# tikv/tikv

Measured on NVIDIA H100. Metric: coprocessor rows/sec (scan+filter+hash-agg) at 1/2/4/8 H100 vs host-CPU ref, higher is better.
Workload: dtype int64

## Files before the change

__graft_entry__.py:

```python
import os
import shutil
import subprocess
import sys

ROOT = os.path.dirname(os.path.abspath(__file__))
CSRC = os.path.join(ROOT, "tikv_b200", "csrc")
OUT_DIR = os.path.join(ROOT, "tikv_b200", "_build")
NVCC = os.environ.get("NVCC", "/usr/local/cuda/bin/nvcc")
NVCC_FLAGS = ["-gencode", "arch=compute_90a,code=sm_90a", "-lineinfo", "-O3", "-std=c++17", "--expt-relaxed-constexpr",
              "-Xcompiler", "-fPIC", "-Xptxas", "-v"]
SOURCES = ["kernels.cu", "encode.cu", "jit.cu", "engine.cu", "sst.cu"]


def _newer(target, deps):
    if not os.path.exists(target):
        return True
    t = os.path.getmtime(target)
    return any(os.path.getmtime(d) > t for d in deps)


def build(verbose=False):
    os.makedirs(OUT_DIR, exist_ok=True)
    headers = [os.path.join(CSRC, f) for f in os.listdir(CSRC) if f.endswith((".h", ".cuh"))] + [os.path.join(ROOT, "include", "b2_copr.h")]
    def compile_one(src):
        s = os.path.join(CSRC, src)
        o = os.path.join(OUT_DIR, src.replace(".cu", ".o"))
        if _newer(o, [s] + headers):
            cmd = [NVCC] + NVCC_FLAGS + ["-c", s, "-o", o]
            r = subprocess.run(cmd, capture_output=True, text=True)
            with open(o + ".log", "w") as f:
                f.write(r.stdout + r.stderr)
            if verbose or r.returncode:
                sys.stderr.write(r.stdout + r.stderr)
            if r.returncode:
                raise RuntimeError(f"nvcc failed for {src}")
        return o

    from concurrent.futures import ThreadPoolExecutor
    with ThreadPoolExecutor(max_workers=len(SOURCES)) as pool:
        objs = list(pool.map(compile_one, SOURCES))
    lib = os.path.join(OUT_DIR, "libb2copr.so")
    if _newer(lib, objs):
        subprocess.check_call([NVCC, "-shared", "-o", lib] + objs + ["-gencode", "arch=compute_90a,code=sm_90a"])
    subprocess.check_call(["make", "-s", "-C", os.path.join(ROOT, "oracle")])
    sys.path.insert(0, ROOT)
    import tikv_b200
    from tikv_b200 import ffi
    ffi.lib()
    _precompile_plans()


def _precompile_plans():
    import ctypes as C
    import threading
    import bench
    from tikv_b200 import ffi, smoke
    L = ffi.lib()
    plans = [bench.build_plan(n) for n in ("c3", "c2", "c4")] + smoke.plans()
    errs = []

    def one(p):
        n = C.c_int32(0)
        if L.b2_plan_precompile(C.byref(p.c), C.byref(n)) != 0:
            errs.append(L.b2_last_error_message().decode())
# ... 21 lines not shown
```

include/b2_copr.h:

```cpp
#ifndef B2_COPR_H_
#define B2_COPR_H_

#ifdef B2_NVRTC
typedef signed char int8_t; typedef unsigned char uint8_t; typedef short int16_t; typedef unsigned short uint16_t;
typedef int int32_t; typedef unsigned int uint32_t; typedef long long int64_t; typedef unsigned long long uint64_t;
#else
#include <stddef.h>
#include <stdint.h>
#endif

#ifdef __cplusplus
extern "C" {
#endif

#define B2_ABI_VERSION 4

enum {
  B2_OK = 0,
  B2_ERR_STORAGE = 1,
  B2_ERR_KEY_IS_LOCKED = 2,
  B2_ERR_WRITE_CONFLICT = 3,
  B2_ERR_EVALUATE = 4,
  B2_ERR_CORRUPTED = 5,
  B2_ERR_DEADLINE = 6,
// ... 250 lines not shown
uint32_t b2_abi_version(void);
const char* b2_build_info(void);

const char* b2_last_error_message(void);

int32_t b2_check_supported(const b2_dag_plan* plan);
int32_t b2_plan_prepare(const b2_dag_plan* plan, int32_t device);
int32_t b2_plan_precompile(const b2_dag_plan* plan, int32_t* n_compiled);
void b2_jit_counters(uint64_t* nvrtc_compiles, uint64_t* disk_cache_hits);

int32_t b2_exec_open(const b2_dag_plan* plan, const b2_key_range* ranges, uint32_t n_ranges,
                     const b2_region_source* src, const b2_exec_config* cfg, b2_exec** out);
int32_t b2_exec_schema(b2_exec* h, int32_t* field_tps, uint32_t* field_flags, uint32_t* n_inout);
int32_t b2_exec_next_batch(b2_exec* h, uint64_t scan_rows, b2_batch* out);
int32_t b2_exec_collect_stats(b2_exec* h, b2_exec_stats* out);
int32_t b2_exec_next_batch_async(b2_exec* h, uint64_t scan_rows);
int32_t b2_exec_poll(b2_exec* h, b2_batch* out);
typedef struct b2_warning {
  int32_t mysql_code;
  int32_t _pad;
  char message[120];
} b2_warning;
int32_t b2_exec_warnings(b2_exec* h, b2_warning* out, uint32_t cap, uint64_t* count_out);
int32_t b2_exec_last_error(b2_exec* h, b2_error_info* out);
enum { B2_ENCODE_TYPE_DEFAULT = 0, B2_ENCODE_TYPE_CHUNK = 1 };
typedef struct b2_encoded_chunk {
  const uint8_t* rows_data;
  uint64_t len;
  uint64_t n_rows;
  int32_t encode_type;
  int32_t location;
} b2_encoded_chunk;
int32_t b2_exec_encode_batch(b2_exec* h, int32_t encode_type, int32_t location, b2_encoded_chunk* out);
int32_t b2_exec_take_scanned_range(b2_exec* h, const uint8_t** lower, uint32_t* lower_len, const uint8_t** upper, uint32_t* upper_len);
int32_t b2_exec_collect_scanned_rows_per_range(b2_exec* h, uint64_t* rows, uint32_t* n_inout);
int32_t b2_exec_can_be_cached(b2_exec* h);
void b2_exec_close(b2_exec* h);

typedef struct b2_agg_partials {
  uint32_t n_groups;
  uint32_t acc_words;
  int32_t location;
  int32_t has_group;
  const uint64_t* keys;
  const uint8_t* key_null;
  const uint64_t* acc;
  uint64_t max_word_mask;
  uint32_t key_words;
  uint32_t _pad;
} b2_agg_partials;
int32_t b2_exec_agg_partials(b2_exec* h, b2_agg_partials* out);
enum { B2_MERGE_ADD = 0, B2_MERGE_MAX = 1, B2_MERGE_OR = 2, B2_MERGE_XOR = 3, B2_MERGE_FIRST_KEY = 4, B2_MERGE_FIRST_VALUE = 5 };
int32_t b2_exec_agg_word_ops(b2_exec* h, uint8_t* ops, uint32_t* n_inout);

int32_t b2_dag_handle(const b2_dag_plan* plan, const b2_key_range* ranges, uint32_t n_ranges,
                      const b2_region_source* src, const b2_exec_config* cfg,
                      b2_batch* out, b2_exec** out_handle);

typedef struct b2_checksum_response {
  uint64_t checksum;
  uint64_t total_kvs;
  uint64_t total_bytes;
} b2_checksum_response;

int32_t b2_checksum_handle(const b2_key_range* ranges, uint32_t n_ranges,
                           const uint8_t* old_prefix, uint32_t old_prefix_len,
                           const uint8_t* new_prefix, uint32_t new_prefix_len,
                           const b2_region_source* src, const b2_exec_config* cfg,
                           b2_checksum_response* out, b2_exec_stats* stats);

int32_t b2_region_pin(int32_t device, uint64_t region_id, uint64_t data_version, const b2_region_source* host_src, b2_region_source* dev_src);
int32_t b2_region_unpin(int32_t device, uint64_t region_id, uint64_t data_version);
void b2_region_cache_stats(int32_t device, uint64_t* bytes_cached, uint64_t* hits, uint64_t* misses);

typedef struct b2_sst_blocks {
  const uint8_t* data;
  const uint64_t* block_offs;
  uint32_t n_blocks;
  uint32_t trailer_len;
  uint32_t key_prefix_len;
  uint32_t key_suffix_len;
} b2_sst_blocks;

typedef struct b2_sst_stats {
  uint64_t n_entries, key_bytes, val_bytes;
  uint64_t n_restart_intervals;
  uint64_t h2d_bytes;
  float decode_ms;
  uint32_t n_lz4_blocks;
} b2_sst_stats;

typedef struct b2_sst b2_sst;
int32_t b2_sst_decode(int32_t device, int32_t location, const b2_sst_blocks* in, b2_sst** h, b2_cf_block* out, b2_sst_stats* stats);
void b2_sst_free(b2_sst* h);
typedef struct b2_sst_encoded {
  const uint8_t* data;
  const uint64_t* block_offs;
  uint64_t data_len;
  uint32_t n_blocks;
  uint32_t _pad;
} b2_sst_encoded;
int32_t b2_sst_encode(int32_t device, const b2_cf_block* flat_device_block, uint32_t entries_per_block, uint32_t restart_interval,
                      uint32_t key_prefix_len, uint8_t key_prefix_byte, uint32_t key_suffix_len, uint32_t trailer_len,
                      b2_sst** h, b2_sst_encoded* out);

int64_t b2_plan_literal(const b2_dag_plan* plan, char* buf, uint64_t cap);
// ... 42 lines not shown
```

tikv_b200/csrc/engine.cu:

```cuda
#include <cuda_runtime.h>
#include <sys/mman.h>
#include <sys/syscall.h>
#include <unistd.h>

#include <algorithm>
#include <cctype>
#include <ctime>
#include <future>
#include <map>
#include <cstdio>
#include <cstring>
#include <memory>
#include <mutex>
#include <string>
#include <vector>

#include <cub/device/device_scan.cuh>

#include "encode.cuh"
#include "jit.h"
#include "kernels.cuh"
#include "plan_literal.h"
#include "plan_compile.h"

// ... 1815 lines not shown
  uint32_t n = (uint32_t)h->cp.output_offsets.size();
  if (field_tps && field_flags)
    for (uint32_t i = 0; i < n && i < *n_inout; ++i) { field_tps[i] = h->cp.schema[h->cp.output_offsets[i]].field_tp; field_flags[i] = h->cp.schema[h->cp.output_offsets[i]].field_flag; }
  *n_inout = n;
  return B2_OK;
}

int32_t b2_exec_next_batch(b2_exec* h, uint64_t scan_rows, b2_batch* out) { return h->next_batch(scan_rows, out); }

int32_t b2_exec_collect_stats(b2_exec* h, b2_exec_stats* out) {
  h->stats.h2d_bytes = h->h2d_bytes; h->stats.d2h_bytes = h->d2h_bytes;
  *out = h->stats;
  return B2_OK;
}
int32_t b2_exec_last_error(b2_exec* h, b2_error_info* out) { *out = h->last_err; return B2_OK; }
int32_t b2_exec_can_be_cached(b2_exec* h) { return (h->check_newer && !h->met_newer_any && !h->saw_lock) ? 1 : 0; }
int32_t b2_exec_take_scanned_range(b2_exec* h, const uint8_t** lower, uint32_t* lower_len, const uint8_t** upper, uint32_t* upper_len) {
  if (!h || !lower || !lower_len || !upper || !upper_len) { g_last_error = "null argument"; return B2_ERR_INVALID_ARG; }
  return h->take_scanned_range(lower, lower_len, upper, upper_len);
}
int32_t b2_exec_collect_scanned_rows_per_range(b2_exec* h, uint64_t* rows, uint32_t* n_inout) {
  if (!h || !n_inout) { g_last_error = "null argument"; return B2_ERR_INVALID_ARG; }
  return h->collect_scanned_rows_per_range(rows, n_inout);
}
int32_t b2_exec_encode_batch(b2_exec* h, int32_t encode_type, int32_t location, b2_encoded_chunk* out) {
  if (!h || !out) { g_last_error = "null argument"; return B2_ERR_INVALID_ARG; }
  return h->encode_batch(encode_type, location, out);
}
void b2_exec_close(b2_exec* h) {
  if (h && h->async_running) h->async_fut.wait();
  delete h;
}

int32_t b2_exec_agg_partials(b2_exec* h, b2_agg_partials* out) {
  if (h->cp.dev.mode != PM_AGG || !h->drained) { g_last_error = "no aggregation state: not an Aggregation pipeline or not drained yet"; return B2_ERR_INVALID_ARG; }
  out->n_groups = h->part_n; out->acc_words = (uint32_t)h->cp.dev.acc_words; out->location = B2_LOC_DEVICE; out->has_group = h->cp.dev.has_group;
  out->keys = (const uint64_t*)h->part_keys; out->key_null = (const uint8_t*)h->part_null; out->acc = (const uint64_t*)h->part_acc;
  out->max_word_mask = 0;
  out->key_words = (uint32_t)std::max(1, h->cp.dev.n_group); out->_pad = 0;
  for (int a = 0; a < h->cp.dev.n_aggs; ++a)
    if (agg_is_extremum(h->cp.dev.aggs[a].kind)) out->max_word_mask |= 1ull << (h->cp.dev.aggs[a].acc_off + 1);
  return B2_OK;
}
int32_t b2_exec_agg_word_ops(b2_exec* h, uint8_t* ops, uint32_t* n_inout) {
  if (!h || !ops || !n_inout) { g_last_error = "null argument"; return B2_ERR_INVALID_ARG; }
  if (h->cp.dev.mode != PM_AGG || !h->drained) { g_last_error = "no aggregation state: not an Aggregation pipeline or not drained yet"; return B2_ERR_INVALID_ARG; }
  const uint32_t n = (uint32_t)h->cp.dev.acc_words;
  if (*n_inout < n) { *n_inout = n; g_last_error = "ops buffer smaller than acc_words"; return B2_ERR_INVALID_ARG; }
  for (uint32_t w = 0; w < n; ++w) ops[w] = (uint8_t)agg_word_op(h->cp.dev, (int)w);
  *n_inout = n;
  return B2_OK;
}

int32_t b2_dag_handle(const b2_dag_plan* plan, const b2_key_range* ranges, uint32_t n_ranges, const b2_region_source* src,
                      const b2_exec_config* cfg, b2_batch* out, b2_exec** out_handle) {
  b2_exec* h = nullptr;
  int rc = b2_exec_open(plan, ranges, n_ranges, src, cfg, &h);
  if (rc) return rc;
  *out_handle = h;
  if (h->paging_size) {
    const uint64_t budget = std::min<uint64_t>(std::max<uint64_t>(h->paging_size * 2, 64), 1ull << 24);
    rc = h->next_batch(budget, out);
    if (rc == B2_OK && out->is_drained == B2_DRAIN_REMAIN) out->is_drained = B2_DRAIN_PAGING;
    return rc;
  }
  return h->next_batch(~0ull, out);
}

int32_t b2_exec_next_batch_async(b2_exec* h, uint64_t scan_rows) {
  if (!h) { g_last_error = "null argument"; return B2_ERR_INVALID_ARG; }
  if (h->async_running) { g_last_error = "a batch is already in flight on this handle"; return B2_ERR_INVALID_ARG; }
  h->async_running = true;
  h->async_fut = std::async(std::launch::async, [h, scan_rows] { return h->next_batch(scan_rows, &h->async_batch); });
  return B2_OK;
}
int32_t b2_exec_poll(b2_exec* h, b2_batch* out) {
  if (!h || !out) { g_last_error = "null argument"; return B2_ERR_INVALID_ARG; }
  if (!h->async_running) { g_last_error = "no batch in flight"; return B2_ERR_INVALID_ARG; }
  if (h->async_fut.wait_for(std::chrono::seconds(0)) != std::future_status::ready) return B2_PENDING;
  const int rc = h->async_fut.get();
  h->async_running = false;
  *out = h->async_batch;
  if (rc) g_last_error = h->last_err.message;
  return rc;
}

int32_t b2_exec_warnings(b2_exec* h, b2_warning* out, uint32_t cap, uint64_t* count_out) {
  if (!h || !count_out) { g_last_error = "null argument"; return B2_ERR_INVALID_ARG; }
  *count_out = h->warnings_total;
  const uint64_t n = std::min<uint64_t>(std::min<uint64_t>(h->warnings_total, cap), 64);
  for (uint64_t i = 0; out && i < n; ++i) {
    out[i].mysql_code = B2_MYSQL_ERR_DIVISION_BY_ZERO; out[i]._pad = 0;
    snprintf(out[i].message, sizeof(out[i].message), "Division by 0");
  }
  return B2_OK;
}

namespace {
struct PinnedRegion {
  std::vector<DevBuf> bufs;
  std::vector<b2_cf_block> write, dflt;
  b2_cf_block lock{};
  std::vector<std::vector<uint8_t>> lock_host;
  std::vector<uint32_t> lock_ko, lock_vo;
  bool has_lock = false;
  uint64_t bytes = 0;
// ... 280 lines not shown
```

tikv_b200/csrc/kernels.cuh:

```cuda
#pragma once
#ifndef B2_NVRTC
#include <cuda_runtime.h>
#endif

#include "b2_device.h"

namespace b2 {

enum { TILE = 256 };

struct Counters {
  unsigned long long err;
  unsigned long long out_rows;
  unsigned long long out_base;
  unsigned long long live_rows;
  unsigned long long processed_keys;
  unsigned long long processed_size;
  unsigned long long entries_scanned;
  unsigned long long default_lookups;
  unsigned long long checksum, total_kvs, total_bytes;
  unsigned int met_newer;
  unsigned int agg_overflow;
  unsigned int n_groups;
  unsigned int bad_prefix;
// ... 87 lines not shown
};

#ifndef B2_NVRTC
cudaError_t launch_scan(const DevPlan& plan, const ScanArgs& a, int grid, size_t smem, cudaStream_t s);
cudaError_t launch_fast(const DevPlan& plan, const ScanArgs& a, int grid, size_t smem, cudaStream_t s);
int fast_max_grid(int mode, size_t smem);
size_t fast_stage_bytes(uint32_t key_cap, uint32_t val_cap);
size_t fast_checksum_bytes();
int scan_max_grid(int mode, size_t smem);
int scan_topn_hbm_max_grid(size_t smem);
cudaError_t launch_scan_topn_hbm(const DevPlan& plan, const ScanArgs& a, int grid, size_t smem, cudaStream_t s);
int scan_num_sms();
size_t scan_stage_bytes(uint32_t key_cap, uint32_t val_cap);
size_t scan_crc_table_bytes();
int scan_kernel_mode(const DevPlan& plan);
size_t scan_out_stage_bytes();
uint32_t scan_stage_entries();
cudaError_t launch_agg_finalize(const DevPlan& plan, const AggTable& t, Counters* ctr, unsigned long long* out_keys, unsigned char* out_key_null,
                                unsigned long long* out_acc, cudaStream_t s);
cudaError_t launch_agg_result(const DevPlan& plan, unsigned int n_groups, const unsigned long long* g_keys, const unsigned char* g_null,
                              const unsigned long long* g_acc, unsigned long long** col_data, unsigned long long** col_bitmap, cudaStream_t s);
cudaError_t launch_topn_merge(const DevPlan& plan, const TopNLists& in, const TopNLists& out, uint32_t fan_in, cudaStream_t s);
cudaError_t launch_topn_gather(const DevPlan& plan, const ScanArgs& a, const TopItem* items, const unsigned int* count, unsigned long long* pay,
                               unsigned char* pay_null, uint32_t stride, cudaStream_t s);
cudaError_t launch_topn_copy(const TopItem* items, const unsigned int* count, uint32_t n_out, uint32_t stride, const unsigned long long* pay0,
                             const unsigned char* null0, const unsigned long long* pay1, const unsigned char* null1, unsigned long long* pay_out,
                             unsigned char* null_out, cudaStream_t s);
cudaError_t launch_topn_merge2(const DevPlan& plan, const TopItem* a, const unsigned int* a_cnt, const TopItem* b, const unsigned int* b_cnt, TopItem* out,
                               unsigned int* out_cnt, uint32_t limit, cudaStream_t s);
cudaError_t launch_pack_nulls(const unsigned char* nulls, uint32_t n_cols, uint32_t stride, uint32_t n, unsigned long long* bitmaps, uint32_t words_per_col, cudaStream_t s);
size_t topn_smem_bytes(uint32_t cap, int n_order);
cudaError_t launch_open_probe(const BlockView* blocks, uint32_t n_wblocks, uint32_t n_blocks, const uint8_t* bounds, const uint32_t* bound_offs, uint32_t n_ranges,
                              uint32_t first_range, uint32_t* out, uint32_t* unit_ok, uint32_t* ends, uint32_t* sample, cudaStream_t s);
cudaError_t launch_gen_sizes(const b2_gen_spec& spec, uint32_t* row_entries, uint32_t* row_val_bytes, cudaStream_t s);
cudaError_t launch_gen_write(const GenArgs& a, cudaStream_t s);
cudaError_t launch_fill_u64(unsigned long long* p, unsigned long long v, size_t n, cudaStream_t s);
enum { MAX_RAW = 16 };
struct RawCol {
  unsigned long long* cells;
  long long* offsets;
  unsigned char* heap;
  unsigned long long* heap_used;
  unsigned long long heap_cap;
};
struct RawArgs {
  RawCol col[MAX_RAW];
  unsigned char var_idx[MAX_RAW], dec_idx[MAX_RAW];
  unsigned int n_var, n_dec;
  const unsigned long long* row_lo; const unsigned long long* row_hi;
  unsigned long long* sums; unsigned long long sums_stride;
  unsigned int* err;
};
cudaError_t launch_raw_materialise(const RawArgs& R, uint64_t max_rows, cudaStream_t s);
cudaError_t launch_reverse_rows(const unsigned long long* in, const unsigned long long* bm_in, uint64_t in_cap, unsigned long long* out, unsigned long long* bm_out,
                                uint64_t out_cap, uint64_t n_rows, uint64_t n_take, uint32_t n_cols, cudaStream_t s);

#endif

}
```

tikv_b200/dist.py:

```python
import torch
import torch.distributed as dist

SIGN = -(1 << 63)


def shard_blocks(n_blocks, world, rank):
    per, rem = divmod(n_blocks, world)
    lo = rank * per + min(rank, rem)
    return list(range(lo, lo + per + (1 if rank < rem else 0)))


def _world():
    return dist.get_world_size() if dist.is_initialized() else 1


def _all_gather_var(t):
    world = _world()
    if world == 1:
        return [t]
    n = torch.tensor([t.shape[0]], dtype=torch.int64, device=t.device)
    sizes = [torch.zeros_like(n) for _ in range(world)]
    dist.all_gather(sizes, n)
    m = int(max(int(s.item()) for s in sizes))
    pad = torch.zeros((m,) + tuple(t.shape[1:]), dtype=t.dtype, device=t.device)
    pad[: t.shape[0]] = t
    out = [torch.zeros_like(pad) for _ in range(world)]
    dist.all_gather(out, pad)
    return [o[: int(s.item())] for o, s in zip(out, sizes)]


F64_ACC_DIGITS = 66


def f64_acc_digits(x):
    import struct
    bits = struct.unpack("<Q", struct.pack("<d", float(x)))[0]
    m, e = bits & ((1 << 52) - 1), (bits >> 52) & 0x7FF
    if e:
        m |= 1 << 52
    else:
        e = 1
    v = (-m if bits >> 63 else m) << (e - 1)
    sign = -1 if v < 0 else 1
    v = abs(v)
    return [sign * ((v >> (32 * i)) & 0xFFFFFFFF) for i in range(F64_ACC_DIGITS)]


def f64_acc_value(words):
    from fractions import Fraction
    total = 0
    for i, w in enumerate(words):
        w = int(w)
        if w >= 1 << 63:
            w -= 1 << 64
        total += w << (32 * i)
    return float(Fraction(total, 1 << 1074))


def merge_agg_partials(keys, key_null, acc, real_words=(), max_words=(), word_ops=None, desc=False):
    from . import ffi
    ops = list(word_ops) if word_ops is not None else []
    max_words = set(max_words) | {w for w, o in enumerate(ops) if o == ffi.MERGE_MAX}
    bit_words = {w: o for w, o in enumerate(ops) if o in (ffi.MERGE_OR, ffi.MERGE_XOR)}
    first_words = [w for w, o in enumerate(ops) if o == ffi.MERGE_FIRST_KEY]
    special = set(real_words) | max_words | set(bit_words) | {w for w, o in enumerate(ops) if o in (ffi.MERGE_FIRST_KEY, ffi.MERGE_FIRST_VALUE)}
    multi = keys.dim() == 2
    kw = keys.shape[1] if multi else 1
    parts = _all_gather_var(torch.cat([keys.view(-1, kw), key_null.to(torch.int64).view(-1, 1), acc], dim=1))
    part_of = torch.cat([torch.full((p.shape[0],), i, dtype=torch.int64, device=p.device) for i, p in enumerate(parts)])
    allp = torch.cat(parts, dim=0)
    if allp.shape[0] == 0:
        return keys[:0], key_null[:0], acc[:0]
    k, nul, a = allp[:, :kw], allp[:, kw], allp[:, kw + 1:]
    if not multi:
        k = torch.where(nul.bool().view(-1, 1), torch.zeros_like(k), k)
    ident = torch.cat([nul.view(-1, 1), k], dim=1)
    uniq, inv = torch.unique(ident, dim=0, return_inverse=True)
    out = torch.zeros((uniq.shape[0], a.shape[1]), dtype=torch.int64, device=a.device)
    ng = uniq.shape[0]
    for w, o in bit_words.items():
        for b0 in range(0, 64, 8):
            shifts = torch.arange(b0, b0 + 8, device=a.device)
            planes = ((a[:, w].view(-1, 1) >> shifts) & 1).to(torch.uint8)
            red = torch.zeros((ng, 8), dtype=torch.uint8, device=a.device)
            if o == ffi.MERGE_OR:
                red.scatter_reduce_(0, inv.view(-1, 1).expand(-1, 8), planes, reduce="amax")
            else:
                red.index_add_(0, inv, planes)
            out[:, w] |= ((red & 1).to(torch.int64) << shifts).sum(dim=1)
    for w in first_words:
        has = a[:, w] != 0
        pref = part_of if desc else len(parts) - 1 - part_of
        pref = torch.where(has, pref, torch.full_like(pref, -1))
        best = torch.full((ng,), -1, dtype=torch.int64, device=a.device).scatter_reduce_(0, inv, pref, reduce="amax")
        cand = has & (pref == best[inv])
        flipped = torch.where(cand, a[:, w] ^ SIGN, torch.full_like(a[:, w], SIGN))
        top = torch.full((ng,), SIGN, dtype=torch.int64, device=a.device).scatter_reduce_(0, inv, flipped, reduce="amax")
        win = cand & (flipped == top[inv])
        out[inv[win], w] = a[win, w]
        out[inv[win], w + 1] = a[win, w + 1]
    int_words = [w for w in range(a.shape[1]) if w not in special]
    if int_words:
        out[:, int_words] = torch.zeros((uniq.shape[0], len(int_words)), dtype=torch.int64, device=a.device).index_add_(0, inv, a[:, int_words])
    for w in real_words:
        s = torch.zeros(uniq.shape[0], dtype=torch.float64, device=a.device).index_add_(0, inv, a[:, w].contiguous().view(torch.float64))
        out[:, w] = s.view(torch.int64)
    for w in max_words:
        flipped = a[:, w] ^ (-(1 << 63))
        m = torch.full((uniq.shape[0],), -(1 << 63), dtype=torch.int64, device=a.device).scatter_reduce_(0, inv, flipped, reduce="amax")
        out[:, w] = m ^ (-(1 << 63))
    if multi:
        return uniq[:, 1:].contiguous(), uniq[:, 0].contiguous(), out
    return uniq[:, 1].contiguous(), uniq[:, 0].bool(), out


def limbs_to_int(lo, hi, unsigned=False):
    lo &= (1 << 64) - 1
    if unsigned:
        hi &= (1 << 64) - 1
    elif hi >= (1 << 63):
        hi -= 1 << 64
    return hi * (1 << 32) + lo


def _order_word(col, null, desc, kind):
# ... 87 lines not shown
```

tikv_b200/ffi.py:

```python
import ctypes as C
import os

_HERE = os.path.dirname(os.path.abspath(__file__))
LIB_PATH = os.path.join(_HERE, "_build", "libb2copr.so")

B2_OK, B2_ERR_STORAGE, B2_ERR_KEY_IS_LOCKED, B2_ERR_WRITE_CONFLICT, B2_ERR_EVALUATE = 0, 1, 2, 3, 4
B2_ERR_CORRUPTED, B2_ERR_DEADLINE, B2_ERR_UNSUPPORTED, B2_ERR_CUDA, B2_ERR_INVALID_ARG = 5, 6, 7, 8, 9
B2_PENDING = 100

TP_TINY, TP_SHORT, TP_LONG, TP_FLOAT, TP_DOUBLE, TP_NULL, TP_TIMESTAMP, TP_LONGLONG, TP_INT24 = 1, 2, 3, 4, 5, 6, 7, 8, 9
TP_DATE, TP_DURATION, TP_DATETIME, TP_YEAR, TP_VARCHAR, TP_BIT = 10, 11, 12, 13, 15, 16
TP_JSON, TP_NEWDECIMAL, TP_ENUM, TP_SET, TP_BLOB, TP_VARSTRING, TP_STRING = 0xF5, 0xF6, 0xF7, 0xF8, 0xFC, 0xFD, 0xFE
FLAG_NOT_NULL, FLAG_UNSIGNED = 1, 32
EXTRA_PHYSICAL_TABLE_ID_COL_ID, EXTRA_COMMIT_TS_COL_ID = -3, -5

LOC_HOST, LOC_DEVICE = 0, 1
ISO_SI, ISO_RC, ISO_RC_CHECK_TS = 0, 1, 2

RPN_CONST_NULL, RPN_CONST_INT, RPN_CONST_UINT, RPN_CONST_REAL, RPN_COLUMN_REF, RPN_FN, RPN_CONST_TIME, RPN_CONST_DURATION, RPN_CONST_BYTES, RPN_CONST_DECIMAL = 0, 1, 2, 3, 4, 5, 6, 7, 8, 9

def _header_enum(prefix):
    import re
    with open(os.path.join(os.path.dirname(_HERE), "include", "b2_copr.h")) as f:
        text = f.read()
# ... 94 lines not shown
    _fields_ = [("status", C.c_int32), ("mysql_code", C.c_int32), ("entry_index", C.c_uint64), ("message", C.c_char * 232)]


class ChecksumResponse(C.Structure):
    _fields_ = [("checksum", C.c_uint64), ("total_kvs", C.c_uint64), ("total_bytes", C.c_uint64)]


class AggPartials(C.Structure):
    _fields_ = [("n_groups", C.c_uint32), ("acc_words", C.c_uint32), ("location", C.c_int32), ("has_group", C.c_int32),
                ("keys", C.c_void_p), ("key_null", C.c_void_p), ("acc", C.c_void_p), ("max_word_mask", C.c_uint64),
                ("key_words", C.c_uint32), ("_pad", C.c_uint32)]


class Warning(C.Structure):
    _fields_ = [("mysql_code", C.c_int32), ("_pad", C.c_int32), ("message", C.c_char * 120)]


class GenSpec(C.Structure):
    _fields_ = [("table_id", C.c_int64), ("first_handle", C.c_uint64), ("n_rows", C.c_uint64), ("n_cols", C.c_uint32),
                ("row_format", C.c_int32), ("seed", C.c_uint64), ("col_lo", C.POINTER(C.c_int64)),
                ("col_range", C.POINTER(C.c_uint64)), ("null_per_million", C.POINTER(C.c_uint32)),
                ("extra_versions_per_million", C.c_uint32), ("delete_per_million", C.c_uint32),
                ("lock_rec_per_million", C.c_uint32), ("commit_ts", C.c_uint64), ("newer_ts", C.c_uint64)]


class GenBlock(C.Structure):
    _fields_ = [("block", CfBlock), ("key_bytes", C.c_uint64), ("val_bytes", C.c_uint64), ("n_user_keys", C.c_uint64)]


class SstBlocks(C.Structure):
    _fields_ = [("data", C.c_void_p), ("block_offs", C.c_void_p), ("n_blocks", C.c_uint32), ("trailer_len", C.c_uint32),
                ("key_prefix_len", C.c_uint32), ("key_suffix_len", C.c_uint32)]


class SstStats(C.Structure):
    _fields_ = [("n_entries", C.c_uint64), ("key_bytes", C.c_uint64), ("val_bytes", C.c_uint64), ("n_restart_intervals", C.c_uint64),
                ("h2d_bytes", C.c_uint64), ("decode_ms", C.c_float), ("n_lz4_blocks", C.c_uint32)]


class SstEncoded(C.Structure):
    _fields_ = [("data", C.c_void_p), ("block_offs", C.c_void_p), ("data_len", C.c_uint64), ("n_blocks", C.c_uint32), ("_pad", C.c_uint32)]


class EncodedChunk(C.Structure):
    _fields_ = [("rows_data", C.c_void_p), ("len", C.c_uint64), ("n_rows", C.c_uint64), ("encode_type", C.c_int32), ("location", C.c_int32)]


ENCODE_TYPE_DEFAULT, ENCODE_TYPE_CHUNK = 0, 1
JIT_AUTO, JIT_SYNC, JIT_OFF = 0, 1, 2

EXPORTED_SYMBOLS = [
    "b2_abi_version", "b2_build_info", "b2_last_error_message", "b2_check_supported", "b2_plan_prepare", "b2_plan_precompile", "b2_jit_counters", "b2_plan_literal", "b2_exec_open", "b2_exec_schema",
    "b2_exec_next_batch", "b2_exec_next_batch_async", "b2_exec_poll", "b2_exec_warnings", "b2_region_pin", "b2_region_unpin", "b2_region_cache_stats", "b2_exec_collect_stats", "b2_exec_last_error", "b2_exec_can_be_cached", "b2_exec_encode_batch", "b2_exec_take_scanned_range", "b2_exec_collect_scanned_rows_per_range", "b2_exec_close",
    "b2_exec_agg_partials", "b2_exec_agg_word_ops", "b2_dag_handle", "b2_checksum_handle", "b2_gen_create", "b2_gen_destroy", "b2_copy_to_host", "b2_copy_to_device",
    "b2_sst_decode", "b2_sst_free", "b2_sst_encode",
    "b2_device_count", "b2_host_alloc_pinned", "b2_host_alloc_pinned_near", "b2_device_numa_node", "b2_host_free_pinned",
]

_lib = None


def lib():
    global _lib
    if _lib is not None:
        return _lib
    if not os.path.exists(LIB_PATH):
        raise RuntimeError(
            f"{LIB_PATH} is missing: the CUDA extension is the product path and there is no CPU fallback. "
            "Run `python -c 'import __graft_entry__ as g; g.build()'` first.")
    L = C.CDLL(LIB_PATH)
    vp, u32, u64, i32 = C.c_void_p, C.c_uint32, C.c_uint64, C.c_int32
    L.b2_abi_version.restype = u32
    L.b2_build_info.restype = C.c_char_p
    L.b2_last_error_message.restype = C.c_char_p
    L.b2_check_supported.argtypes = [C.POINTER(DagPlan)]
    L.b2_check_supported.restype = i32
    L.b2_plan_prepare.argtypes = [C.POINTER(DagPlan), i32]
    L.b2_plan_prepare.restype = i32
    L.b2_plan_precompile.argtypes = [C.POINTER(DagPlan), C.POINTER(i32)]
    L.b2_plan_precompile.restype = i32
    L.b2_jit_counters.argtypes = [C.POINTER(u64), C.POINTER(u64)]
    L.b2_jit_counters.restype = None
    L.b2_exec_open.argtypes = [C.POINTER(DagPlan), C.POINTER(KeyRange), u32, C.POINTER(RegionSource), C.POINTER(ExecConfig), C.POINTER(vp)]
    L.b2_exec_open.restype = i32
    L.b2_exec_schema.argtypes = [vp, C.POINTER(i32), C.POINTER(u32), C.POINTER(u32)]
    L.b2_exec_schema.restype = i32
    L.b2_exec_next_batch.argtypes = [vp, u64, C.POINTER(Batch)]
    L.b2_exec_next_batch.restype = i32
    L.b2_exec_next_batch_async.argtypes = [vp, u64]
    L.b2_exec_next_batch_async.restype = i32
    L.b2_exec_poll.argtypes = [vp, C.POINTER(Batch)]
    L.b2_exec_poll.restype = i32
    L.b2_exec_warnings.argtypes = [vp, C.POINTER(Warning), u32, C.POINTER(u64)]
    L.b2_exec_warnings.restype = i32
    L.b2_region_pin.argtypes = [i32, u64, u64, C.POINTER(RegionSource), C.POINTER(RegionSource)]
    L.b2_region_pin.restype = i32
    L.b2_region_unpin.argtypes = [i32, u64, u64]
    L.b2_region_unpin.restype = i32
    L.b2_region_cache_stats.argtypes = [i32, C.POINTER(u64), C.POINTER(u64), C.POINTER(u64)]
    L.b2_region_cache_stats.restype = None
    L.b2_exec_collect_stats.argtypes = [vp, C.POINTER(ExecStats)]
    L.b2_exec_collect_stats.restype = i32
    L.b2_exec_last_error.argtypes = [vp, C.POINTER(ErrorInfo)]
    L.b2_exec_last_error.restype = i32
    L.b2_exec_encode_batch.argtypes = [vp, i32, i32, C.POINTER(EncodedChunk)]
    L.b2_exec_encode_batch.restype = i32
    L.b2_exec_take_scanned_range.argtypes = [vp, C.POINTER(C.c_void_p), C.POINTER(C.c_uint32), C.POINTER(C.c_void_p), C.POINTER(C.c_uint32)]
    L.b2_exec_take_scanned_range.restype = i32
    L.b2_exec_collect_scanned_rows_per_range.argtypes = [vp, C.POINTER(C.c_uint64), C.POINTER(C.c_uint32)]
    L.b2_exec_collect_scanned_rows_per_range.restype = i32
    L.b2_exec_can_be_cached.argtypes = [vp]
    L.b2_exec_can_be_cached.restype = i32
    L.b2_exec_agg_partials.argtypes = [vp, C.POINTER(AggPartials)]
    L.b2_exec_agg_partials.restype = i32
    L.b2_exec_agg_word_ops.argtypes = [vp, C.POINTER(C.c_uint8), C.POINTER(u32)]
    L.b2_exec_agg_word_ops.restype = i32
    L.b2_exec_close.argtypes = [vp]
    L.b2_exec_close.restype = None
    L.b2_dag_handle.argtypes = [C.POINTER(DagPlan), C.POINTER(KeyRange), u32, C.POINTER(RegionSource), C.POINTER(ExecConfig), C.POINTER(Batch), C.POINTER(vp)]
    L.b2_dag_handle.restype = i32
    L.b2_checksum_handle.argtypes = [C.POINTER(KeyRange), u32, C.c_char_p, u32, C.c_char_p, u32, C.POINTER(RegionSource), C.POINTER(ExecConfig), C.POINTER(ChecksumResponse), C.POINTER(ExecStats)]
    L.b2_checksum_handle.restype = i32
    L.b2_gen_create.argtypes = [i32, C.POINTER(GenSpec), C.POINTER(vp), C.POINTER(GenBlock)]
    L.b2_gen_create.restype = i32
    L.b2_gen_destroy.argtypes = [vp]
    L.b2_gen_destroy.restype = None
    L.b2_sst_decode.argtypes = [i32, i32, C.POINTER(SstBlocks), C.POINTER(vp), C.POINTER(CfBlock), C.POINTER(SstStats)]
    L.b2_sst_decode.restype = i32
    L.b2_sst_free.argtypes = [vp]
    L.b2_sst_free.restype = None
    L.b2_sst_encode.argtypes = [i32, C.POINTER(CfBlock), u32, u32, u32, C.c_uint8, u32, u32, C.POINTER(vp), C.POINTER(SstEncoded)]
    L.b2_sst_encode.restype = i32
    L.b2_copy_to_host.argtypes = [i32, vp, vp, u64]
    L.b2_copy_to_host.restype = i32
    L.b2_copy_to_device.argtypes = [i32, vp, vp, u64]
    L.b2_copy_to_device.restype = i32
    L.b2_device_count.restype = i32
    L.b2_host_alloc_pinned.argtypes = [u64]
    L.b2_host_alloc_pinned.restype = vp
    L.b2_host_alloc_pinned_near.argtypes = [i32, u64]
    L.b2_host_alloc_pinned_near.restype = vp
    L.b2_device_numa_node.argtypes = [i32]
    L.b2_device_numa_node.restype = i32
    L.b2_host_free_pinned.argtypes = [vp]
    L.b2_host_free_pinned.restype = None
    if L.b2_abi_version() != 4:
        raise RuntimeError("libb2copr ABI version mismatch")
    _lib = L
    return L
```

Before: 38.62 billion.

## Merge aggregation partials on device with a native sort-based kernel

Adds a native CUDA path for merging per-device hash-aggregation partials. It radix-sorts rows by their key words (LSD passes), flags group heads, scans to assign group ids, and reduces each group with a warp, including FIRST key/value selection. This replaces the multi-step torch merge whenever the data is on the GPU and no real words are present. It adds several kernel launches, per-call buffer allocation and a host sync in exchange for cutting torch op overhead.

Result: faster. 40.25 billion (median of 6 runs) (+4.2%).

```diff
diff --git a/__graft_entry__.py b/__graft_entry__.py
--- a/__graft_entry__.py
+++ b/__graft_entry__.py
@@ -9,7 +9,7 @@
 NVCC = os.environ.get("NVCC", "/usr/local/cuda/bin/nvcc")
 NVCC_FLAGS = ["-gencode", "arch=compute_90a,code=sm_90a", "-lineinfo", "-O3", "-std=c++17", "--expt-relaxed-constexpr",
               "-Xcompiler", "-fPIC", "-Xptxas", "-v"]
-SOURCES = ["kernels.cu", "encode.cu", "jit.cu", "engine.cu", "sst.cu"]
+SOURCES = ["kernels.cu", "encode.cu", "jit.cu", "engine.cu", "sst.cu", "agg_merge.cu"]
 
 
 def _newer(target, deps):
diff --git a/include/b2_copr.h b/include/b2_copr.h
--- a/include/b2_copr.h
+++ b/include/b2_copr.h
@@ -326,6 +326,10 @@
 int32_t b2_exec_agg_partials(b2_exec* h, b2_agg_partials* out);
 enum { B2_MERGE_ADD = 0, B2_MERGE_MAX = 1, B2_MERGE_OR = 2, B2_MERGE_XOR = 3, B2_MERGE_FIRST_KEY = 4, B2_MERGE_FIRST_VALUE = 5 };
 int32_t b2_exec_agg_word_ops(b2_exec* h, uint8_t* ops, uint32_t* n_inout);
+int32_t b2_agg_merge(int32_t device, uint64_t cuda_stream, uint64_t n_rows, uint32_t key_words, uint32_t acc_words,
+                     const int64_t* keys, uint64_t keys_stride, const uint8_t* key_null, const int64_t* acc, uint64_t acc_stride,
+                     const uint64_t* part_offs, uint32_t n_parts, const uint8_t* ops, int32_t desc,
+                     int64_t* out_keys, uint8_t* out_null, int64_t* out_acc, uint64_t* n_groups);
 
 int32_t b2_dag_handle(const b2_dag_plan* plan, const b2_key_range* ranges, uint32_t n_ranges,
                       const b2_region_source* src, const b2_exec_config* cfg,
diff --git a/tikv_b200/csrc/agg_merge.cu b/tikv_b200/csrc/agg_merge.cu
--- /dev/null
+++ b/tikv_b200/csrc/agg_merge.cu
@@ -0,0 +1,158 @@
+#include <cub/device/device_radix_sort.cuh>
+#include <cub/device/device_scan.cuh>
+
+#include <algorithm>
+
+#include "kernels.cuh"
+
+namespace b2 {
+
+namespace {
+
+__global__ void agg_merge_gather_kernel(AggMergeArgs a, uint32_t word, const unsigned int* perm, unsigned int* perm_out, long long* keys_out) {
+  const uint32_t i = blockIdx.x * blockDim.x + threadIdx.x;
+  if (i >= a.n) return;
+  unsigned int r = i;
+  if (perm) r = perm[i];
+  else perm_out[i] = i;
+  long long v;
+  if (word == a.key_words) v = a.key_null[r];
+  else if (a.key_words == 1 && a.key_null[r]) v = 0;
+  else v = a.keys[(size_t)r * a.keys_stride + word];
+  keys_out[i] = v;
+}
+
+__device__ __forceinline__ bool agg_merge_same_ident(const AggMergeArgs& a, unsigned int r, unsigned int q) {
+  if (a.key_null[r] != a.key_null[q]) return false;
+  if (a.key_words == 1 && a.key_null[r]) return true;
+  for (uint32_t k = 0; k < a.key_words; ++k)
+    if (a.keys[(size_t)r * a.keys_stride + k] != a.keys[(size_t)q * a.keys_stride + k]) return false;
+  return true;
+}
+
+__global__ void agg_merge_heads_kernel(AggMergeArgs a, const unsigned int* perm, unsigned int* flags) {
+  const uint32_t i = blockIdx.x * blockDim.x + threadIdx.x;
+  if (i >= a.n) return;
+  flags[i] = i == 0 || !agg_merge_same_ident(a, perm[i], perm[i - 1]);
+}
+
+__global__ void agg_merge_starts_kernel(const unsigned int* gid, uint32_t n, unsigned int* starts, unsigned int* n_groups) {
+  const uint32_t i = blockIdx.x * blockDim.x + threadIdx.x;
+  if (i >= n) return;
+  const unsigned int g = gid[i];
+  if (g != (i ? gid[i - 1] : 0u)) starts[g - 1] = i;
+  if (i == n - 1) { starts[g] = n; *n_groups = g; }
+}
+
+__device__ __forceinline__ uint32_t agg_merge_part_of(const unsigned long long* part_offs, uint32_t n_parts, unsigned int r) {
+  uint32_t lo = 0, hi = n_parts;
+  while (hi - lo > 1) {
+    const uint32_t mid = (lo + hi) / 2;
+    if (part_offs[mid] <= r) lo = mid; else hi = mid;
+  }
+  return lo;
+}
+
+__device__ __forceinline__ unsigned long long agg_merge_op(unsigned char op, unsigned long long x, unsigned long long y) {
+  if (op == B2_MERGE_ADD) return x + y;
+  if (op == B2_MERGE_MAX) return x > y ? x : y;
+  if (op == B2_MERGE_OR) return x | y;
+  return x ^ y;
+}
+
+__global__ void agg_merge_reduce_kernel(AggMergeArgs a, const unsigned int* perm, const unsigned int* starts, const unsigned int* n_groups) {
+  const uint32_t lane = threadIdx.x & 31, n_warps = gridDim.x * blockDim.x / 32, ng = *n_groups;
+  for (uint32_t g = (blockIdx.x * blockDim.x + threadIdx.x) / 32; g < ng; g += n_warps) {
+    const uint32_t lo = starts[g], hi = starts[g + 1];
+    if (lane == 0) {
+      const long long* first = a.keys + (size_t)perm[lo] * a.keys_stride;
+      const unsigned char mask = a.key_null[perm[lo]];
+      for (uint32_t k = 0; k < a.key_words; ++k) a.out_keys[(size_t)g * a.key_words + k] = (a.key_words == 1 && mask != 0) ? 0 : first[k];
+      a.out_null[g] = mask;
+    }
+    long long* out = a.out_acc + (size_t)g * a.acc_words;
+    for (uint32_t w = 0; w < a.acc_words; ++w) {
+      const long long* col = a.acc + w;
+      const unsigned char op = a.ops[w];
+      if (op == B2_MERGE_FIRST_VALUE) continue;
+      if (op == B2_MERGE_FIRST_KEY) {
+        uint32_t has = 0, pref = 0, pos = 0;
+        unsigned long long key = 0;
+        for (uint32_t j = lo + lane; j < hi; j += 32) {
+          const unsigned long long k = (unsigned long long)col[(size_t)perm[j] * a.acc_stride];
+          if (k == 0) continue;
+          const uint32_t p = agg_merge_part_of(a.part_offs, a.n_parts, perm[j]), pr = a.desc ? p : a.n_parts - 1 - p;
+          if (!has || pr > pref || (pr == pref && k >= key)) { has = 1; pref = pr; key = k; pos = j; }
+        }
+        for (int off = 16; off; off >>= 1) {
+          const uint32_t h2 = __shfl_down_sync(0xffffffffu, has, off), p2 = __shfl_down_sync(0xffffffffu, pref, off), j2 = __shfl_down_sync(0xffffffffu, pos, off);
+          const unsigned long long k2 = __shfl_down_sync(0xffffffffu, key, off);
+          if (h2 && (!has || p2 > pref || (p2 == pref && (k2 > key || (k2 == key && j2 > pos))))) { has = 1; pref = p2; key = k2; pos = j2; }
+        }
+        if (lane == 0) {
+          out[w] = has ? (long long)key : 0;
+          out[w + 1] = has ? col[(size_t)perm[pos] * a.acc_stride + 1] : 0;
+        }
+        continue;
+      }
+      unsigned long long acc = 0;
+      for (uint32_t j = lo + lane; j < hi; j += 32) acc = agg_merge_op(op, acc, (unsigned long long)col[(size_t)perm[j] * a.acc_stride]);
+      for (int off = 16; off; off >>= 1) acc = agg_merge_op(op, acc, __shfl_down_sync(0xffffffffu, acc, off));
+      if (lane == 0) out[w] = (long long)acc;
+    }
+  }
+}
+
+size_t align256(size_t x) { return (x + 255) & ~(size_t)255; }
+
+}
+
+cudaError_t launch_agg_merge(const AggMergeArgs& a, void* tmp, size_t* tmp_bytes, cudaStream_t s) {
+  const uint32_t n = a.n;
+  const size_t keys_b = align256((size_t)n * 8), idx_b = align256((size_t)n * 4), starts_b = align256(((size_t)n + 1) * 4);
+  const size_t fixed = 2 * keys_b + 3 * idx_b + starts_b;
+  cub::DoubleBuffer<long long> kq(nullptr, nullptr);
+  cub::DoubleBuffer<unsigned int> vq(nullptr, nullptr);
+  if (!tmp) {
+    size_t sort_key_b = 0, sort_mask_b = 0, scan_b = 0;
+    cudaError_t e = cub::DeviceRadixSort::SortPairs(nullptr, sort_key_b, kq, vq, (int)n, 0, 64, s);
+    if (e == cudaSuccess) e = cub::DeviceRadixSort::SortPairs(nullptr, sort_mask_b, kq, vq, (int)n, 0, (int)a.key_words, s);
+    if (e == cudaSuccess) e = cub::DeviceScan::InclusiveSum(nullptr, scan_b, (unsigned int*)nullptr, (unsigned int*)nullptr, (int)n, s);
+    *tmp_bytes = fixed + std::max(std::max(sort_key_b, sort_mask_b), scan_b);
+    return e;
+  }
+  if (*tmp_bytes < fixed) return cudaErrorInvalidValue;
+  const size_t cub_b = *tmp_bytes - fixed;
+  cudaError_t e = cudaSuccess;
+  if (n == 0) return cudaMemsetAsync(a.n_groups, 0, 4, s);
+
+  char* p = (char*)tmp;
+  long long* k0 = (long long*)p; p += keys_b;
+  long long* k1 = (long long*)p; p += keys_b;
+  unsigned int* v0 = (unsigned int*)p; p += idx_b;
+  unsigned int* v1 = (unsigned int*)p; p += idx_b;
+  unsigned int* gid = (unsigned int*)p; p += idx_b;
+  unsigned int* starts = (unsigned int*)p; p += starts_b;
+  void* cub_tmp = p;
+  kq = cub::DoubleBuffer<long long>(k0, k1);
+  vq = cub::DoubleBuffer<unsigned int>(v0, v1);
+  const int threads = 256, blocks = (int)((n + threads - 1) / threads);
+  for (uint32_t pass = 0; pass <= a.key_words; ++pass) {
+    const uint32_t word = pass < a.key_words ? a.key_words - 1 - pass : a.key_words;
+    agg_merge_gather_kernel<<<blocks, threads, 0, s>>>(a, word, pass ? vq.Current() : nullptr, vq.Current(), kq.Current());
+    size_t b = cub_b;
+    e = cub::DeviceRadixSort::SortPairs(cub_tmp, b, kq, vq, (int)n, 0, word == a.key_words ? (int)a.key_words : 64, s);
+    if (e != cudaSuccess) return e;
+  }
+  const unsigned int* perm = vq.Current();
+  agg_merge_heads_kernel<<<blocks, threads, 0, s>>>(a, perm, gid);
+  size_t b = cub_b;
+  e = cub::DeviceScan::InclusiveSum(cub_tmp, b, gid, gid, (int)n, s);
+  if (e != cudaSuccess) return e;
+  agg_merge_starts_kernel<<<blocks, threads, 0, s>>>(gid, n, starts, a.n_groups);
+  const int reduce_blocks = (int)(((size_t)n * 32 + threads - 1) / threads < 4096 ? ((size_t)n * 32 + threads - 1) / threads : 4096);
+  agg_merge_reduce_kernel<<<reduce_blocks, threads, 0, s>>>(a, perm, starts, a.n_groups);
+  return cudaGetLastError();
+}
+
+}
diff --git a/tikv_b200/csrc/engine.cu b/tikv_b200/csrc/engine.cu
--- a/tikv_b200/csrc/engine.cu
+++ b/tikv_b200/csrc/engine.cu
@@ -1891,6 +1891,65 @@
   return B2_OK;
 }
 
+int32_t b2_agg_merge(int32_t device, uint64_t cuda_stream, uint64_t n_rows, uint32_t key_words, uint32_t acc_words,
+                     const int64_t* keys, uint64_t keys_stride, const uint8_t* key_null, const int64_t* acc, uint64_t acc_stride,
+                     const uint64_t* part_offs, uint32_t n_parts, const uint8_t* ops, int32_t desc,
+                     int64_t* out_keys, uint8_t* out_null, int64_t* out_acc, uint64_t* n_groups) {
+  if (!part_offs || !n_groups || (acc_words && !ops) ||
+      (n_rows && (!keys || !key_null || !out_keys || !out_null || (acc_words && (!acc || !out_acc))))) {
+    g_last_error = "null argument"; return B2_ERR_INVALID_ARG;
+  }
+  if (key_words < 1 || key_words > 4 || n_rows >= (1ull << 31) || n_parts < 1 || part_offs[0] != 0 || part_offs[n_parts] != n_rows ||
+      keys_stride < key_words || (acc_words && acc_stride < acc_words)) {
+    g_last_error = "b2_agg_merge: 1..4 key words, n_rows < 2^31, n_parts >= 1 offsets from 0 to n_rows, row strides >= the words of a row";
+    return B2_ERR_INVALID_ARG;
+  }
+  for (uint32_t p = 0; p < n_parts; ++p)
+    if (part_offs[p] > part_offs[p + 1]) { g_last_error = "b2_agg_merge: part offsets decrease"; return B2_ERR_INVALID_ARG; }
+  for (uint32_t w = 0; w < acc_words; ++w) {
+    const bool pair_ok = ops[w] == B2_MERGE_FIRST_KEY ? w + 1 < acc_words && ops[w + 1] == B2_MERGE_FIRST_VALUE
+                       : ops[w] == B2_MERGE_FIRST_VALUE ? w > 0 && ops[w - 1] == B2_MERGE_FIRST_KEY : ops[w] <= B2_MERGE_XOR;
+    if (!pair_ok) { g_last_error = "b2_agg_merge: unknown op, or a FIRST key word not followed by its value word"; return B2_ERR_INVALID_ARG; }
+  }
+  *n_groups = 0;
+  if (n_rows == 0) return B2_OK;
+  int prev = -1;
+  cudaGetDevice(&prev);
+  if (cudaSetDevice(device) != cudaSuccess) { g_last_error = "cudaSetDevice failed (the CUDA device path is required; there is no CPU fallback)"; return B2_ERR_CUDA; }
+  struct RestoreDevice { int d; ~RestoreDevice() { if (d >= 0) cudaSetDevice(d); } } restore{prev};
+  const cudaStream_t s = (cudaStream_t)cuda_stream;
+  AggMergeArgs a{};
+  a.keys = (const long long*)keys; a.key_null = key_null; a.acc = (const long long*)acc;
+  a.keys_stride = keys_stride; a.acc_stride = acc_stride; a.n = (uint32_t)n_rows; a.key_words = key_words; a.acc_words = acc_words; a.n_parts = n_parts;
+  a.desc = desc; a.out_keys = (long long*)out_keys; a.out_null = out_null; a.out_acc = (long long*)out_acc;
+  const size_t ops_b = (acc_words + 7) & ~7u, offs_b = ((size_t)n_parts + 1) * 8, up_b = ops_b + offs_b;
+  const size_t count_off = (up_b + 255) & ~(size_t)255, scratch_off = count_off + 256;
+  size_t merge_b = 0;
+  cudaError_t e = launch_agg_merge(a, nullptr, &merge_b, s);
+  HostBuf host;
+  DevBuf dev;
+  if (e == cudaSuccess) e = host.reserve(up_b + 8);
+  if (e == cudaSuccess) e = dev.reserve(scratch_off + merge_b);
+  if (e != cudaSuccess) { g_last_error = std::string("b2_agg_merge buffers: ") + cudaGetErrorString(e); return B2_ERR_CUDA; }
+  uint8_t* hp = (uint8_t*)host.p;
+  if (acc_words) memcpy(hp, ops, acc_words);
+  memcpy(hp + ops_b, part_offs, offs_b);
+  uint8_t* dp = (uint8_t*)dev.p;
+  a.ops = dp; a.part_offs = (const unsigned long long*)(dp + ops_b);
+  a.n_groups = (unsigned int*)(dp + count_off);
+  e = cudaMemcpyAsync(dp, hp, up_b, cudaMemcpyHostToDevice, s);
+  if (e == cudaSuccess) e = launch_agg_merge(a, dp + scratch_off, &merge_b, s);
+  if (e == cudaSuccess) e = cudaMemcpyAsync(hp + up_b, a.n_groups, 4, cudaMemcpyDeviceToHost, s);
+  if (e == cudaSuccess) e = cudaStreamSynchronize(s);
+  if (e != cudaSuccess) {
+    cudaStreamSynchronize(s);
+    g_last_error = std::string("b2_agg_merge: ") + cudaGetErrorString(e);
+    return B2_ERR_CUDA;
+  }
+  *n_groups = *(const unsigned int*)(hp + up_b);
+  return B2_OK;
+}
+
 int32_t b2_dag_handle(const b2_dag_plan* plan, const b2_key_range* ranges, uint32_t n_ranges, const b2_region_source* src,
                       const b2_exec_config* cfg, b2_batch* out, b2_exec** out_handle) {
   b2_exec* h = nullptr;
diff --git a/tikv_b200/csrc/kernels.cuh b/tikv_b200/csrc/kernels.cuh
--- a/tikv_b200/csrc/kernels.cuh
+++ b/tikv_b200/csrc/kernels.cuh
@@ -163,6 +163,21 @@
   unsigned int* err;
 };
 cudaError_t launch_raw_materialise(const RawArgs& R, uint64_t max_rows, cudaStream_t s);
+struct AggMergeArgs {
+  const long long* keys;
+  const unsigned char* key_null;
+  const long long* acc;
+  uint64_t keys_stride, acc_stride;
+  uint32_t n, key_words, acc_words, n_parts;
+  const unsigned char* ops;
+  const unsigned long long* part_offs;
+  int32_t desc;
+  long long* out_keys;
+  unsigned char* out_null;
+  long long* out_acc;
+  unsigned int* n_groups;
+};
+cudaError_t launch_agg_merge(const AggMergeArgs& a, void* tmp, size_t* tmp_bytes, cudaStream_t s);
 cudaError_t launch_reverse_rows(const unsigned long long* in, const unsigned long long* bm_in, uint64_t in_cap, unsigned long long* out, unsigned long long* bm_out,
                                 uint64_t out_cap, uint64_t n_rows, uint64_t n_take, uint32_t n_cols, cudaStream_t s);
 
diff --git a/tikv_b200/dist.py b/tikv_b200/dist.py
--- a/tikv_b200/dist.py
+++ b/tikv_b200/dist.py
@@ -58,19 +58,60 @@
 
 
 def merge_agg_partials(keys, key_null, acc, real_words=(), max_words=(), word_ops=None, desc=False):
+    multi = keys.dim() == 2
+    kw = keys.shape[1] if multi else 1
+    if keys.is_cuda and not real_words:
+        if _world() == 1:
+            return _merge_native(keys.view(-1, kw), key_null, acc, [keys.shape[0]], multi, max_words, word_ops, desc)
+        parts = _all_gather_var(torch.cat([keys.view(-1, kw), key_null.to(torch.int64).view(-1, 1), acc], dim=1))
+        allp = torch.cat(parts, dim=0)
+        return _merge_native(allp[:, :kw], allp[:, kw], allp[:, kw + 1:], [p.shape[0] for p in parts], multi, max_words, word_ops, desc)
+    parts = _all_gather_var(torch.cat([keys.view(-1, kw), key_null.to(torch.int64).view(-1, 1), acc], dim=1))
+    return _merge_gathered_torch(parts, kw, multi, real_words, max_words, word_ops, desc)
+
+
+def _merge_native(keys, key_null, acc, part_sizes, multi, max_words=(), word_ops=None, desc=False):
+    import ctypes as C
+    from . import ffi
+    if keys.stride(1) != 1:
+        keys = keys.contiguous()
+    if acc.shape[1] and acc.stride(1) != 1:
+        acc = acc.contiguous()
+    if key_null.dtype not in (torch.bool, torch.uint8) or not key_null.is_contiguous():
+        key_null = key_null.to(torch.uint8).contiguous()
+    n, kw, aw = keys.shape[0], keys.shape[1], acc.shape[1]
+    ops = list(word_ops) if word_ops is not None else [ffi.MERGE_ADD] * aw
+    for w in max_words:
+        ops[w] = ffi.MERGE_MAX
+    offs = [0]
+    for m in part_sizes:
+        offs.append(offs[-1] + m)
+    out_k = torch.empty((n, kw) if multi else (n,), dtype=torch.int64, device=keys.device)
+    out_n = torch.empty(n, dtype=torch.uint8, device=keys.device)
+    out_a = torch.empty((n, aw), dtype=torch.int64, device=keys.device)
+    ng = C.c_uint64()
+    L = ffi.lib()
+    rc = L.b2_agg_merge(keys.device.index, torch.cuda.current_stream(keys.device).cuda_stream, n, kw, aw,
+                        keys.data_ptr(), keys.stride(0), key_null.data_ptr(), acc.data_ptr(), acc.stride(0) if aw else 0,
+                        (C.c_uint64 * len(offs))(*offs), len(part_sizes), (C.c_uint8 * max(1, aw))(*ops), int(bool(desc)),
+                        out_k.data_ptr(), out_n.data_ptr(), out_a.data_ptr(), C.byref(ng))
+    if rc != 0:
+        raise RuntimeError("b2_agg_merge: " + L.b2_last_error_message().decode())
+    g = ng.value
+    return out_k[:g], (out_n[:g].to(torch.int64) if multi else out_n[:g].view(torch.bool)), out_a[:g]
+
+
+def _merge_gathered_torch(parts, kw, multi, real_words=(), max_words=(), word_ops=None, desc=False):
     from . import ffi
     ops = list(word_ops) if word_ops is not None else []
     max_words = set(max_words) | {w for w, o in enumerate(ops) if o == ffi.MERGE_MAX}
     bit_words = {w: o for w, o in enumerate(ops) if o in (ffi.MERGE_OR, ffi.MERGE_XOR)}
     first_words = [w for w, o in enumerate(ops) if o == ffi.MERGE_FIRST_KEY]
     special = set(real_words) | max_words | set(bit_words) | {w for w, o in enumerate(ops) if o in (ffi.MERGE_FIRST_KEY, ffi.MERGE_FIRST_VALUE)}
-    multi = keys.dim() == 2
-    kw = keys.shape[1] if multi else 1
-    parts = _all_gather_var(torch.cat([keys.view(-1, kw), key_null.to(torch.int64).view(-1, 1), acc], dim=1))
     part_of = torch.cat([torch.full((p.shape[0],), i, dtype=torch.int64, device=p.device) for i, p in enumerate(parts)])
     allp = torch.cat(parts, dim=0)
     if allp.shape[0] == 0:
-        return keys[:0], key_null[:0], acc[:0]
+        return (allp[:, :kw], allp[:, kw], allp[:, kw + 1:]) if multi else (allp[:, 0], allp[:, 1].bool(), allp[:, 2:])
     k, nul, a = allp[:, :kw], allp[:, kw], allp[:, kw + 1:]
     if not multi:
         k = torch.where(nul.bool().view(-1, 1), torch.zeros_like(k), k)
diff --git a/tikv_b200/ffi.py b/tikv_b200/ffi.py
--- a/tikv_b200/ffi.py
+++ b/tikv_b200/ffi.py
@@ -170,7 +170,7 @@
 EXPORTED_SYMBOLS = [
     "b2_abi_version", "b2_build_info", "b2_last_error_message", "b2_check_supported", "b2_plan_prepare", "b2_plan_precompile", "b2_jit_counters", "b2_plan_literal", "b2_exec_open", "b2_exec_schema",
     "b2_exec_next_batch", "b2_exec_next_batch_async", "b2_exec_poll", "b2_exec_warnings", "b2_region_pin", "b2_region_unpin", "b2_region_cache_stats", "b2_exec_collect_stats", "b2_exec_last_error", "b2_exec_can_be_cached", "b2_exec_encode_batch", "b2_exec_take_scanned_range", "b2_exec_collect_scanned_rows_per_range", "b2_exec_close",
-    "b2_exec_agg_partials", "b2_exec_agg_word_ops", "b2_dag_handle", "b2_checksum_handle", "b2_gen_create", "b2_gen_destroy", "b2_copy_to_host", "b2_copy_to_device",
+    "b2_exec_agg_partials", "b2_exec_agg_word_ops", "b2_agg_merge", "b2_dag_handle", "b2_checksum_handle", "b2_gen_create", "b2_gen_destroy", "b2_copy_to_host", "b2_copy_to_device",
     "b2_sst_decode", "b2_sst_free", "b2_sst_encode",
     "b2_device_count", "b2_host_alloc_pinned", "b2_host_alloc_pinned_near", "b2_device_numa_node", "b2_host_free_pinned",
 ]
@@ -233,6 +233,8 @@
     L.b2_exec_agg_partials.restype = i32
     L.b2_exec_agg_word_ops.argtypes = [vp, C.POINTER(C.c_uint8), C.POINTER(u32)]
     L.b2_exec_agg_word_ops.restype = i32
+    L.b2_agg_merge.argtypes = [i32, u64, u64, u32, u32, vp, u64, vp, vp, u64, C.POINTER(u64), u32, C.POINTER(C.c_uint8), i32, vp, vp, vp, C.POINTER(u64)]
+    L.b2_agg_merge.restype = i32
     L.b2_exec_close.argtypes = [vp]
     L.b2_exec_close.restype = None
     L.b2_dag_handle.argtypes = [C.POINTER(DagPlan), C.POINTER(KeyRange), u32, C.POINTER(RegionSource), C.POINTER(ExecConfig), C.POINTER(Batch), C.POINTER(vp)]
```
